# YuanxunLu/LiveSpeechPortraits

Hardware: NVIDIA H100
Metric: 512x512 frames/sec (Feature2Face_G large / May.yaml) (higher is better)
Workload: dtype fp16 hi+lo split operands (3 wgmma MMAs per K step), fp32 accumulate

## Files before the change

livespeechportraits_b200/csrc/conv_wgmma.cuh:

```cuda
#pragma once
#include <cuda_bf16.h>
#include <cuda_fp16.h>
#include "ptx.cuh"

namespace lspg {

constexpr int kTileM = 128;
constexpr int kChunk = 64;
constexpr int kATile = kTileM * 128;
constexpr int kMaxTaps = 9;
constexpr int kThreads = 384;
constexpr int kSmemBudget = 227 * 1024;

struct FastDiv {
  uint32_t mul, shr, d;
};
inline FastDiv make_fast_div(uint32_t d) {
  FastDiv f;
  f.d = d; f.mul = 0; f.shr = 0;
  if (d > 1) {
    uint32_t l = 0;
    while ((1u << l) < d) ++l;
    const uint64_t pw = 31 + l;
    f.mul = static_cast<uint32_t>(((1ull << pw) + d - 1) / d);
    f.shr = static_cast<uint32_t>(pw - 32);
  }
  return f;
}
__device__ __forceinline__ int fast_div(int n, const FastDiv& f) {
  return f.d == 1 ? n : static_cast<int>(__umulhi(static_cast<uint32_t>(n), f.mul) >> f.shr);
}

struct alignas(64) ConvParams {
  const float* scale;
  const float* shift;
  __nv_bfloat16* out_ptr;
  const __nv_bfloat16* res_ptr;
  long long out_limb_stride;
  long long res_limb_stride;
  float* out_f32;
  uint8_t* out_u8;
  float* partial;
  unsigned long long* trace;
  int32_t out_channels, res_channels;
  int32_t out_up;
  int32_t relu, has_res;
  int32_t batch, hs, ws;
  int32_t tw_log2, th_log2;
  int32_t total_tiles;
  int32_t n_split, tiles_per_split;
  int32_t n_tiles;
  int32_t tiles_x, tiles_y, tiles_n;
  int32_t n_phases;
  int32_t trace_skip;
  FastDiv fd_tps, fd_m_tiles, fd_n_tiles, fd_tiles_x, fd_tiles_y;
  int32_t n_taps, n_src;
  int32_t chunks[2];
  int32_t split_len;
  int32_t patch_w, patch_h;
  int32_t desc_base_offset;
  int8_t patch_dx0[4], patch_dy0[4];
  int16_t tap_row[4][kMaxTaps];
  int8_t tap_map[4][kMaxTaps];
  int8_t tap_dx[4][kMaxTaps];
  int8_t tap_dy[4][kMaxTaps];
  CUtensorMap a[4];
  CUtensorMap w;
};

constexpr int kBarBytes = 1024;
constexpr int kTailStride = 17;
template <bool TAIL>
struct AuxCfg {
  static constexpr int kTailBytes = TAIL ? kTileM * kTailStride * 4 : 0;
  static constexpr int kBytes = kBarBytes + kTailBytes;
};

template <int BN, int NL, bool TAIL>
struct ConvCfg {
  using Aux = AuxCfg<TAIL>;
  static constexpr int kBTile = BN * 128;
  static constexpr int kStage = NL * (kATile + kBTile);
  static constexpr int kAvail = kSmemBudget - 1024  - Aux::kBytes;
  static constexpr int kStagesRaw = kAvail / kStage;
  static constexpr int kStages = kStagesRaw > 8 ? 8 : kStagesRaw;
  static constexpr int kSmemBytes = 1024 + kStages * kStage + Aux::kBytes;
  static_assert(kStages >= 2, "pipeline needs at least two stages");
  static_assert(BN == 16 || BN == 64 || BN == 128, "instantiated N tiles");
};

constexpr int kTraceTiles = 12;
constexpr int kTraceSlots = 4 + 8 * kTraceTiles + 4;

struct TileCoord {
  int z, nt, x0, y0, n0, split;
};

__device__ __forceinline__ void trace_stamp(const ConvParams& p, int slot) {
  if (p.trace != nullptr && slot < kTraceSlots) p.trace[static_cast<size_t>(blockIdx.x) * kTraceSlots + slot] = clock64();
}
__device__ __forceinline__ void trace_time(const ConvParams& p, bool at_exit) {
  if (p.trace != nullptr) {
    unsigned long long ns;
    asm volatile("mov.u64 %0, %globaltimer;" : "=l"(ns));
    unsigned long long* t = p.trace + static_cast<size_t>(blockIdx.x) * kTraceSlots;
    t[at_exit ? 3 : 2] = ns;
    if (at_exit) t[4 + 8 * kTraceTiles] = clock64();
  }
}
__device__ __forceinline__ void trace_tile(const ConvParams& p, int lt, int k) {
  if (p.trace != nullptr) {
    const int i = lt - p.trace_skip;
    if (i >= 0 && i < kTraceTiles) p.trace[static_cast<size_t>(blockIdx.x) * kTraceSlots + 4 + 8 * i + k] = clock64();
  }
}

__device__ __forceinline__ TileCoord decode_tile(const ConvParams& p, int t) {
  TileCoord c;
  c.split = fast_div(t, p.fd_tps);
  t -= c.split * p.tiles_per_split;
  const int r = fast_div(t, p.fd_m_tiles);
  const int mt = t - r * static_cast<int>(p.fd_m_tiles.d);
  c.z = fast_div(r, p.fd_n_tiles);
  c.nt = r - c.z * p.n_tiles;
  const int r2 = fast_div(mt, p.fd_tiles_x);
  const int tx = mt - r2 * p.tiles_x;
  const int tn = fast_div(r2, p.fd_tiles_y);
  const int ty = r2 - tn * p.tiles_y;
  c.x0 = tx << p.tw_log2;
  c.y0 = ty << p.th_log2;
  c.n0 = tn << (7 - p.tw_log2 - p.th_log2);
  return c;
}

__device__ __forceinline__ uint32_t pack_bf16x2(float lo, float hi) {
  __nv_bfloat162 v = __floats2bfloat162_rn(lo, hi);
  return *reinterpret_cast<uint32_t*>(&v);
}
__device__ __forceinline__ float bf16_lo(uint32_t u) { return __uint_as_float(u << 16); }
__device__ __forceinline__ float bf16_hi(uint32_t u) { return __uint_as_float(u & 0xFFFF0000u); }

template <bool F16>
__device__ __forceinline__ uint32_t pack2(float lo, float hi) {
  if constexpr (F16) {
    uint32_t r;
    asm("cvt.rn.satfinite.f16x2.f32 %0, %1, %2;" : "=r"(r) : "f"(hi), "f"(lo));
    return r;
  } else {
    return pack_bf16x2(lo, hi);
  }
}
template <bool F16>
__device__ __forceinline__ float unpack_lo(uint32_t u) {
  if constexpr (F16) return __half2float(__ushort_as_half(static_cast<unsigned short>(u & 0xFFFFu)));
  else return bf16_lo(u);
}
template <bool F16>
__device__ __forceinline__ float unpack_hi(uint32_t u) {
  if constexpr (F16) return __half2float(__ushort_as_half(static_cast<unsigned short>(u >> 16)));
  else return bf16_hi(u);
}

__device__ __forceinline__ void row_pixel(const ConvParams& p, const TileCoord& tc, int row, int& n, int& y, int& x) {
  x = tc.x0 + (row & ((1 << p.tw_log2) - 1));
  y = tc.y0 + ((row >> p.tw_log2) & ((1 << p.th_log2) - 1));
  n = tc.n0 + (row >> (p.tw_log2 + p.th_log2));
}

template <int BN, int NL, bool TAIL>
__device__ __forceinline__ void epilogue_regs(const ConvParams& p, const float (&acc)[BN / 2], const TileCoord& tc, int t, int cw,
                                              float* tail_stg) {
  const int wtid = threadIdx.x & 127;
  const int warp = wtid >> 5, lane = wtid & 31;
  const int r0 = cw * 64 + warp * 16 + (lane >> 2);
  const int c0 = 2 * (lane & 3);
  if constexpr (TAIL) {
    float* stg = tail_stg + cw * 64 * kTailStride;
    ptx::named_bar_sync(1 + cw, 128);
#pragma unroll
    for (int j = 0; j < BN / 8; ++j)
#pragma unroll
      for (int h = 0; h < 2; ++h) {
        float* s = stg + (r0 - cw * 64 + 8 * h) * kTailStride + 8 * j + c0;
        s[0] = acc[4 * j + 2 * h];
        s[1] = acc[4 * j + 2 * h + 1];
      }
    ptx::named_bar_sync(1 + cw, 128);
    if (wtid >= 64) return;
    const int row = cw * 64 + wtid;
    const float* v = stg + wtid * kTailStride;
    int pn, py_, px_;
    row_pixel(p, tc, row, pn, py_, px_);
    if (pn >= p.batch || py_ >= p.hs || px_ >= p.ws) return;
    const int oh = 2 * p.hs, ow = 2 * p.ws;
    if (p.out_u8 != nullptr) {
#pragma unroll
      for (int py = 0; py < 2; ++py) {
        uint8_t b[6];
#pragma unroll
        for (int px = 0; px < 2; ++px)
#pragma unroll
          for (int c = 0; c < 3; ++c) {
            const int col = (py * 2 + px) * 3 + c;
            const float vf = tanhf(v[col] * __ldg(p.scale + col) + __ldg(p.shift + col));
            float u = __fmul_rn(__fmul_rn(__fadd_rn(vf, 1.0f), 0.5f), 255.0f);
            u = fminf(fmaxf(u, 0.0f), 255.0f);
            b[px * 3 + c] = static_cast<uint8_t>(static_cast<int>(u));
          }
        uint8_t* dst = p.out_u8 + ((static_cast<size_t>(pn) * oh + (2 * py_ + py)) * ow + 2 * px_) * 3;
        uint16_t* d16 = reinterpret_cast<uint16_t*>(dst);
        d16[0] = static_cast<uint16_t>(b[0] | (b[1] << 8));
        d16[1] = static_cast<uint16_t>(b[2] | (b[3] << 8));
        d16[2] = static_cast<uint16_t>(b[4] | (b[5] << 8));
      }
    } else {
#pragma unroll
      for (int c = 0; c < 3; ++c) {
#pragma unroll
        for (int py = 0; py < 2; ++py) {
          const int c0_ = (py * 2 + 0) * 3 + c, c1_ = (py * 2 + 1) * 3 + c;
          float2 o;
          o.x = tanhf(v[c0_] * __ldg(p.scale + c0_) + __ldg(p.shift + c0_));
          o.y = tanhf(v[c1_] * __ldg(p.scale + c1_) + __ldg(p.shift + c1_));
          float* dst = p.out_f32 + ((static_cast<size_t>(pn) * 3 + c) * oh + (2 * py_ + py)) * ow + 2 * px_;
          *reinterpret_cast<float2*>(dst) = o;
        }
      }
    }
  } else {
    if (p.n_split > 1) {
#pragma unroll
      for (int h = 0; h < 2; ++h) {
        float* dst = p.partial + (static_cast<size_t>(t) * kTileM + r0 + 8 * h) * BN + c0;
#pragma unroll
        for (int j = 0; j < BN / 8; ++j)
          *reinterpret_cast<float2*>(dst + 8 * j) = make_float2(acc[4 * j + 2 * h], acc[4 * j + 2 * h + 1]);
      }
      return;
    }
#pragma unroll
    for (int h = 0; h < 2; ++h) {
      int pn, py_, px_;
      row_pixel(p, tc, r0 + 8 * h, pn, py_, px_);
      if (pn >= p.batch || py_ >= p.hs || px_ >= p.ws) continue;
      const int oh = p.out_up ? 2 * p.hs : p.hs, ow = p.out_up ? 2 * p.ws : p.ws;
      const int oy = p.out_up ? 2 * py_ + (tc.z >> 1) : py_, ox = p.out_up ? 2 * px_ + (tc.z & 1) : px_;
      __nv_bfloat16* out_row = p.out_ptr + ((static_cast<size_t>(pn) * oh + oy) * ow + ox) * p.out_channels + tc.nt * BN + c0;
      const __nv_bfloat16* res_row =
          p.has_res ? p.res_ptr + ((static_cast<size_t>(pn) * p.hs + py_) * p.ws + px_) * p.res_channels + tc.nt * BN + c0 : nullptr;
      const float* sc = p.scale + tc.nt * BN + c0;
      const float* sf = p.shift + tc.nt * BN + c0;
      uint32_t rw[NL][BN / 8];
      if (p.has_res) {
#pragma unroll
        for (int l = 0; l < NL; ++l)
#pragma unroll
          for (int j = 0; j < BN / 8; ++j)
            rw[l][j] = __ldg(reinterpret_cast<const unsigned int*>(res_row + l * p.res_limb_stride + 8 * j));
      }
#pragma unroll
      for (int j = 0; j < BN / 8; ++j) {
        const float2 s2 = __ldg(reinterpret_cast<const float2*>(sc + 8 * j));
        const float2 f2 = __ldg(reinterpret_cast<const float2*>(sf + 8 * j));
        float y0 = fmaf(acc[4 * j + 2 * h], s2.x, f2.x);
        float y1 = fmaf(acc[4 * j + 2 * h + 1], s2.y, f2.y);
        if (p.has_res) {
#pragma unroll
          for (int l = 0; l < NL; ++l) {
            y0 += unpack_lo<NL == 2>(rw[l][j]);
            y1 += unpack_hi<NL == 2>(rw[l][j]);
          }
        }
// ... 68 lines not shown
      }
      __syncwarp();
    }
    ptx::pdl_wait();
    int stage = 0;
    uint32_t phase = 0;
    int issued = 0;
    int lt = 0;
    for (int t = t0; t < p.total_tiles; t += tstep, ++lt) {
      const TileCoord tc = decode_tile(p, t);
      const int kb0 = tc.split * p.split_len;
      const int kb1 = (kb0 + p.split_len < num_kb) ? kb0 + p.split_len : num_kb;
      if (lane == 0) trace_tile(p, lt, 6);
      for (int kb = kb0; kb < kb1; ++kb, ++issued) {
        const int tap = kb / kb_per_tap;
        const int rem = kb - tap * kb_per_tap;
        const int s = (rem < p.chunks[0]) ? 0 : 1;
        const int c = s ? rem - p.chunks[0] : rem;
        const int amap = p.tap_map[tc.z][tap];
        const int xx = tc.x0 + p.tap_dx[tc.z][tap];
        const int yy = tc.y0 + p.tap_dy[tc.z][tap];
        const bool early = issued < pre;
        if (!early) ptx::mbar_wait(&empty_bar[stage], phase ^ 1);
        if (ptx::elect_one()) {
          uint8_t* st = smem + stage * Cfg::kStage;
          if (!early) ptx::mbar_expect_tx(&full_bar[stage], Cfg::kStage);
#pragma unroll
          for (int l = 0; l < NL; ++l) {
            ptx::tma_load_5d(&p.a[amap + s], &full_bar[stage], st + l * kATile, c * kChunk, xx, yy, tc.n0, l);
            if (!early)
              ptx::tma_load_3d(&p.w, &full_bar[stage], st + NL * kATile + l * Cfg::kBTile, kb * kChunk, tc.nt * BN,
                               l * p.n_phases + tc.z);
          }
        }
        __syncwarp();
        if (++stage == Cfg::kStages) { stage = 0; phase ^= 1; }
      }
      if (lane == 0) trace_tile(p, lt, 7);
    }
  } else if (warp >= 4) {
    ptx::pdl_wait();
    const int cw = (warp >> 2) - 1;
    const bool wg_leader = (threadIdx.x & 127) == 0;
    int stage = 0;
    uint32_t phase = 0;
    int lt = 0;
    for (int t = t0; t < p.total_tiles; t += tstep, ++lt) {
      const TileCoord tc = decode_tile(p, t);
      const int kb0 = tc.split * p.split_len;
      const int kb1 = (kb0 + p.split_len < num_kb) ? kb0 + p.split_len : num_kb;
      if (threadIdx.x == 128) trace_tile(p, lt, 0);
      float acc[BN / 2];
#pragma unroll
      for (int i = 0; i < BN / 2; ++i) acc[i] = 0.0f;
      int prev = -1;
      for (int kb = kb0; kb < kb1; ++kb) {
        ptx::mbar_wait(&full_bar[stage], phase);
        if (threadIdx.x == 128 && kb == kb0) trace_tile(p, lt, 1);
        ptx::wgmma_fence();
        const uint32_t a0 = ptx::smem_u32(smem + stage * Cfg::kStage) + cw * 64 * 128;
        const uint32_t b0 = ptx::smem_u32(smem + stage * Cfg::kStage) + NL * kATile;
        const uint64_t a_hi = ptx::gmma_desc_sw128(a0);
        const uint64_t b_hi = ptx::gmma_desc_sw128(b0);
#pragma unroll
        for (int k = 0; k < kChunk / 16; ++k) {
          const uint32_t accum = (kb > kb0 || k > 0) ? 1u : 0u;
          ptx::wgmma_m64k16<BN, NL == 2>(acc, a_hi + 2 * k, b_hi + 2 * k, accum);
          if constexpr (NL == 2) {
            const uint64_t a_lo = ptx::gmma_desc_sw128(a0 + kATile);
            const uint64_t b_lo = ptx::gmma_desc_sw128(b0 + Cfg::kBTile);
            ptx::wgmma_m64k16<BN, true>(acc, a_hi + 2 * k, b_lo + 2 * k, 1u);
            ptx::wgmma_m64k16<BN, true>(acc, a_lo + 2 * k, b_hi + 2 * k, 1u);
          }
        }
        ptx::wgmma_commit();
        ptx::wgmma_wait<1>();
        if (prev >= 0 && wg_leader) release_stage<1>(&empty_bar[prev]);
        prev = stage;
        if (++stage == Cfg::kStages) { stage = 0; phase ^= 1; }
      }
      ptx::wgmma_wait<0>();
      if (prev >= 0 && wg_leader) release_stage<1>(&empty_bar[prev]);
      if (threadIdx.x == 128) trace_tile(p, lt, 2);
      epilogue_regs<BN, NL, TAIL>(p, acc, tc, t, cw, tail_stg);
      if (threadIdx.x == 128) trace_tile(p, lt, 3);
    }
  }
  if (threadIdx.x == 0) trace_time(p, true);
}


constexpr int kPatchSlot = 23 * 1024;
constexpr int kPatchStride = 23 * 1024;

template <int BN, int NL, bool TAIL>
struct PatchCfg {
  using Aux = AuxCfg<TAIL>;
  static constexpr int kBTile = BN * 128;
  static constexpr int kTPS = TAIL ? 9 : (BN >= 128 ? (NL == 1 ? 2 : 1) : (NL == 1 ? 3 : 2));
  static constexpr int kAStage = NL * kPatchStride;
  static constexpr int kBStage = NL * kTPS * kBTile;
  static constexpr int kAStages = 2;
  static constexpr int kAvail = kSmemBudget - 1024 - Aux::kBytes - kAStages * kAStage;
  static constexpr int kBStagesRaw = kAvail / kBStage;
  static constexpr int kBStages = kBStagesRaw > 12 ? 12 : kBStagesRaw;
  static constexpr int kSmemBytes = 1024 + kAStages * kAStage + kBStages * kBStage + Aux::kBytes;
  static_assert(kBStages >= 2, "B ring needs at least two stages");
  static_assert(BN == 16 || BN == 64 || BN == 128, "instantiated N tiles");
};

template <int BN, int NL, bool TAIL, int CL>
__global__ void __launch_bounds__(kThreads, 1) conv_patch_kernel(const __grid_constant__ ConvParams p) {
  using Cfg = PatchCfg<BN, NL, TAIL>;
  const int t0 = static_cast<int>(blockIdx.x), tstep = static_cast<int>(gridDim.x);
  extern __shared__ uint8_t smem_raw[];
  uint8_t* smem = reinterpret_cast<uint8_t*>((reinterpret_cast<uintptr_t>(smem_raw) + 1023) & ~uintptr_t(1023));
  uint8_t* a_ring = smem;
  uint8_t* b_ring = a_ring + Cfg::kAStages * Cfg::kAStage;
  uint8_t* aux = b_ring + Cfg::kBStages * Cfg::kBStage;
  uint64_t* afull_bar = reinterpret_cast<uint64_t*>(aux);
  uint64_t* aempty_bar = afull_bar + Cfg::kAStages;
  uint64_t* bfull_bar = aempty_bar + Cfg::kAStages;
  uint64_t* bempty_bar = bfull_bar + Cfg::kBStages;
  float* tail_stg = reinterpret_cast<float*>(aux + kBarBytes);

  const int warp = __shfl_sync(0xffffffffu, static_cast<int>(threadIdx.x >> 5), 0);
  const int lane = threadIdx.x & 31;
  if (threadIdx.x == 0) { trace_stamp(p, 0); trace_time(p, false); }

  if (warp == 0 && lane == 0) {
    for (int i = 0; i < 4; ++i) ptx::prefetch_tmap(&p.a[i]);
    ptx::prefetch_tmap(&p.w);
    for (int i = 0; i < Cfg::kAStages; ++i) { ptx::mbar_init(&afull_bar[i], 1); ptx::mbar_init(&aempty_bar[i], 2); }
    for (int i = 0; i < Cfg::kBStages; ++i) { ptx::mbar_init(&bfull_bar[i], 1); ptx::mbar_init(&bempty_bar[i], 2 * CL); }
    ptx::fence_mbar_init();
  }
  __syncthreads();
  if (CL > 1) ptx::cluster_sync();
  const uint32_t crank = (CL > 1) ? ptx::cluster_ctarank() : 0u;
  constexpr uint16_t kMask = static_cast<uint16_t>((1u << CL) - 1u);
  ptx::pdl_launch_dependents();
  if (threadIdx.x == 0) trace_stamp(p, 1);

  int kb_per_tap = 0;
  for (int s = 0; s < p.n_src; ++s) kb_per_tap += p.chunks[s];
  const int patch_bytes = p.patch_w * p.patch_h * 128;
  const int n_groups = (p.n_taps + Cfg::kTPS - 1) / Cfg::kTPS;

  if (warp == 0) {
    ptx::pdl_wait();
    int ia = 0, ib = 0;
    uint32_t pha = 0, phb = 0;
    int a_tile = t0, a_ci = -1;
    auto issue_a = [&]() {
      if (a_tile >= p.total_tiles) return;
      const TileCoord tc = decode_tile(p, a_tile);
      const int ci0 = tc.split * p.split_len;
      const int ci1 = (ci0 + p.split_len < kb_per_tap) ? ci0 + p.split_len : kb_per_tap;
      if (a_ci < 0) a_ci = ci0;
      const int s = (a_ci < p.chunks[0]) ? 0 : 1;
      const int c = (s == 0) ? a_ci : a_ci - p.chunks[0];
      ptx::mbar_wait(&aempty_bar[ia], pha ^ 1);
      if (ptx::elect_one()) {
        ptx::mbar_expect_tx(&afull_bar[ia], NL * patch_bytes);
#pragma unroll
        for (int l = 0; l < NL; ++l)
          ptx::tma_load_5d(&p.a[s], &afull_bar[ia], a_ring + ia * Cfg::kAStage + l * kPatchStride, c * kChunk,
                           tc.x0 + p.patch_dx0[tc.z], tc.y0 + p.patch_dy0[tc.z], tc.n0, l);
      }
      __syncwarp();
      if (++ia == Cfg::kAStages) { ia = 0; pha ^= 1; }
      if (++a_ci == ci1) { a_ci = -1; a_tile += tstep; }
    };
    issue_a();
    const int a_after_group = (n_groups > 1) ? 1 : 0;
    int lt = 0;
    for (int t = t0; t < p.total_tiles; t += tstep, ++lt) {
      const TileCoord tc = decode_tile(p, t);
      const int ci0 = tc.split * p.split_len;
      const int ci1 = (ci0 + p.split_len < kb_per_tap) ? ci0 + p.split_len : kb_per_tap;
      if (lane == 0) trace_tile(p, lt, 6);
      for (int ci = ci0; ci < ci1; ++ci) {
        for (int g = 0; g < n_groups; ++g) {
          ptx::mbar_wait(&bempty_bar[ib], phb ^ 1);
          if (ptx::elect_one()) {
            uint8_t* st = b_ring + ib * Cfg::kBStage;
            if constexpr (CL == 1 && NL == 1) {
              ptx::mbar_expect_tx(&bfull_bar[ib], Cfg::kBStage);
              ptx::tma_load_4d(&p.w, &bfull_bar[ib], st, ci * kChunk, tc.nt * BN, g * Cfg::kTPS, tc.z);
            } else {
              const int tap0 = g * Cfg::kTPS;
              const int ntap = (tap0 + Cfg::kTPS < p.n_taps) ? Cfg::kTPS : p.n_taps - tap0;
              ptx::mbar_expect_tx(&bfull_bar[ib], NL * ntap * Cfg::kBTile);
              constexpr int kRows = BN / CL;
              for (int ti = 0; ti < ntap; ++ti)
#pragma unroll
                for (int l = 0; l < NL; ++l) {
                  uint8_t* dst = st + (ti * NL + l) * Cfg::kBTile + crank * kRows * 128;
                  if constexpr (CL == 1)
                    ptx::tma_load_4d(&p.w, &bfull_bar[ib], dst, ci * kChunk, tc.nt * BN, tap0 + ti, l * p.n_phases + tc.z);
                  else
                    ptx::tma_load_4d_mc(&p.w, &bfull_bar[ib], dst, ci * kChunk, tc.nt * BN + crank * kRows, tap0 + ti,
                                        l * p.n_phases + tc.z, kMask);
                }
            }
          }
          __syncwarp();
          if (++ib == Cfg::kBStages) { ib = 0; phb ^= 1; }
          if (g == a_after_group) issue_a();
        }
      }
      if (lane == 0) trace_tile(p, lt, 7);
    }
  } else if (warp >= 4) {
    ptx::pdl_wait();
    const int cw = (warp >> 2) - 1;
    const bool wg_leader = (threadIdx.x & 127) == 0;
    int ia = 0, ib = 0;
    uint32_t pha = 0, phb = 0;
    const uint32_t sbo = static_cast<uint32_t>(p.patch_w) * 128u;
    const uint32_t row_off = static_cast<uint32_t>(cw * 8 * p.patch_w) * 128u;
    const bool boff = p.desc_base_offset != 0;
    int lt = 0;
    for (int t = t0; t < p.total_tiles; t += tstep, ++lt) {
      const TileCoord tc = decode_tile(p, t);
      const int ci0 = tc.split * p.split_len;
      const int ci1 = (ci0 + p.split_len < kb_per_tap) ? ci0 + p.split_len : kb_per_tap;
      if (threadIdx.x == 128) trace_tile(p, lt, 0);
      float acc[BN / 2];
#pragma unroll
      for (int i = 0; i < BN / 2; ++i) acc[i] = 0.0f;
      int prev_b = -1, prev_a = -1;
      for (int ci = ci0; ci < ci1; ++ci) {
        ptx::mbar_wait(&afull_bar[ia], pha);
        const uint32_t a0 = ptx::smem_u32(a_ring + ia * Cfg::kAStage) + row_off;
        for (int g = 0; g < n_groups; ++g) {
          ptx::mbar_wait(&bfull_bar[ib], phb);
          if (threadIdx.x == 128 && ci == ci0 && g == 0) trace_tile(p, lt, 1);
          ptx::wgmma_fence();
          const int tap0 = g * Cfg::kTPS;
          const int tap1 = (tap0 + Cfg::kTPS < p.n_taps) ? tap0 + Cfg::kTPS : p.n_taps;
          const uint32_t b0 = ptx::smem_u32(b_ring + ib * Cfg::kBStage);
          for (int tap = tap0; tap < tap1; ++tap) {
            const uint32_t a_hi_addr = a0 + static_cast<uint32_t>(p.tap_row[tc.z][tap]) * 128u;
            const uint32_t b_hi_addr = b0 + static_cast<uint32_t>(tap - tap0) * (NL * Cfg::kBTile);
            const uint64_t a_hi = ptx::gmma_desc_sw128(a_hi_addr, sbo, boff);
            const uint64_t b_hi = ptx::gmma_desc_sw128(b_hi_addr);
#pragma unroll
            for (int k = 0; k < kChunk / 16; ++k) {
              const uint32_t accum = (ci > ci0 || tap > 0 || k > 0) ? 1u : 0u;
              ptx::wgmma_m64k16<BN, NL == 2>(acc, a_hi + 2 * k, b_hi + 2 * k, accum);
              if constexpr (NL == 2) {
                const uint64_t a_lo = ptx::gmma_desc_sw128(a_hi_addr + kPatchStride, sbo, boff);
                const uint64_t b_lo = ptx::gmma_desc_sw128(b_hi_addr + Cfg::kBTile);
                ptx::wgmma_m64k16<BN, true>(acc, a_hi + 2 * k, b_lo + 2 * k, 1u);
                ptx::wgmma_m64k16<BN, true>(acc, a_lo + 2 * k, b_hi + 2 * k, 1u);
              }
            }
          }
          ptx::wgmma_commit();
          ptx::wgmma_wait<1>();
          if (wg_leader) {
            if (prev_b >= 0) release_stage<CL>(&bempty_bar[prev_b]);
            if (prev_a >= 0) ptx::mbar_arrive(&aempty_bar[prev_a]);
          }
          prev_b = ib;
          prev_a = (g == n_groups - 1) ? ia : -1;
          if (++ib == Cfg::kBStages) { ib = 0; phb ^= 1; }
        }
        if (++ia == Cfg::kAStages) { ia = 0; pha ^= 1; }
      }
      ptx::wgmma_wait<0>();
      if (wg_leader) {
        if (prev_b >= 0) release_stage<CL>(&bempty_bar[prev_b]);
        if (prev_a >= 0) ptx::mbar_arrive(&aempty_bar[prev_a]);
      }
      if (threadIdx.x == 128) trace_tile(p, lt, 2);
      epilogue_regs<BN, NL, TAIL>(p, acc, tc, t, cw, tail_stg);
      if (threadIdx.x == 128) trace_tile(p, lt, 3);
    }
  }
  if (CL > 1) ptx::cluster_sync();
  if (threadIdx.x == 0) trace_time(p, true);
}

struct ReduceParams {
  const float* partial;
  const float* scale;
  const float* shift;
  const __nv_bfloat16* res;
  long long res_limb_stride;
  __nv_bfloat16* out;
  long long out_limb_stride;
  int32_t n_split, tiles_per_split, m_tiles, n_tiles, n_phases;
  int32_t tiles_x, tiles_y, tw_log2, th_log2, bn;
  int32_t batch, hs, ws, up, channels, relu, has_res, nl;
};

__global__ void __launch_bounds__(128) splitk_reduce_kernel(const ReduceParams p) {
  ptx::pdl_wait();
  ptx::pdl_launch_dependents();
  const int groups = p.bn >> 2;
  const long long total = static_cast<long long>(p.tiles_per_split) * kTileM * groups;
  for (long long e = blockIdx.x * static_cast<long long>(blockDim.x) + threadIdx.x; e < total;
       e += static_cast<long long>(gridDim.x) * blockDim.x) {
    const int g = static_cast<int>(e % groups);
    const long long r0 = e / groups;
    const int row = static_cast<int>(r0 % kTileM);
    const int tile = static_cast<int>(r0 / kTileM);
    const int mt = tile % p.m_tiles;
    const int r1 = tile / p.m_tiles;
    const int nt = r1 % p.n_tiles;
    const int z = r1 / p.n_tiles;
    const int tx = mt % p.tiles_x;
    const int r2 = mt / p.tiles_x;
    const int ty = r2 % p.tiles_y;
    const int tn = r2 / p.tiles_y;
    const int tw = row & ((1 << p.tw_log2) - 1);
    const int th = (row >> p.tw_log2) & ((1 << p.th_log2) - 1);
    const int nb = row >> (p.tw_log2 + p.th_log2);
    const int n = (tn << (7 - p.tw_log2 - p.th_log2)) + nb;
    const int y = (ty << p.th_log2) + th, x = (tx << p.tw_log2) + tw;
    if (n >= p.batch || y >= p.hs || x >= p.ws) continue;
    float acc[4] = {0.f, 0.f, 0.f, 0.f};
    const size_t split_stride = static_cast<size_t>(p.tiles_per_split) * kTileM * p.bn;
    const float* src0 = p.partial + (static_cast<size_t>(tile) * kTileM + row) * p.bn + g * 4;
    int s = 0;
    for (; s + 16 <= p.n_split; s += 16) {
      float4 v[16];
#pragma unroll
      for (int u = 0; u < 16; ++u) v[u] = *reinterpret_cast<const float4*>(src0 + (s + u) * split_stride);
#pragma unroll
      for (int u = 0; u < 16; ++u) {
        acc[0] += v[u].x; acc[1] += v[u].y; acc[2] += v[u].z; acc[3] += v[u].w;
      }
    }
    for (; s + 4 <= p.n_split; s += 4) {
      float4 v[4];
#pragma unroll
      for (int u = 0; u < 4; ++u) v[u] = *reinterpret_cast<const float4*>(src0 + (s + u) * split_stride);
#pragma unroll
      for (int u = 0; u < 4; ++u) { acc[0] += v[u].x; acc[1] += v[u].y; acc[2] += v[u].z; acc[3] += v[u].w; }
    }
    for (; s < p.n_split; ++s) {
      const float4 a = *reinterpret_cast<const float4*>(src0 + s * split_stride);
      acc[0] += a.x; acc[1] += a.y; acc[2] += a.z; acc[3] += a.w;
    }
    const int ch = nt * p.bn + g * 4;
    const int oh = p.up ? 2 * p.hs : p.hs, ow = p.up ? 2 * p.ws : p.ws;
    const int oy = p.up ? 2 * y + (z >> 1) : y, ox = p.up ? 2 * x + (z & 1) : x;
    const size_t off = ((static_cast<size_t>(n) * oh + oy) * ow + ox) * p.channels + ch;
    const float4 sc = *reinterpret_cast<const float4*>(p.scale + ch), sh = *reinterpret_cast<const float4*>(p.shift + ch);
    float yv[4] = {fmaf(acc[0], sc.x, sh.x), fmaf(acc[1], sc.y, sh.y), fmaf(acc[2], sc.z, sh.z), fmaf(acc[3], sc.w, sh.w)};
    if (p.has_res) {
      for (int l = 0; l < p.nl; ++l) {
        const uint2 r = *reinterpret_cast<const uint2*>(p.res + l * p.res_limb_stride + off);
        if (p.nl == 2) {
          yv[0] += unpack_lo<true>(r.x); yv[1] += unpack_hi<true>(r.x); yv[2] += unpack_lo<true>(r.y); yv[3] += unpack_hi<true>(r.y);
        } else {
          yv[0] += bf16_lo(r.x); yv[1] += bf16_hi(r.x); yv[2] += bf16_lo(r.y); yv[3] += bf16_hi(r.y);
        }
      }
// ... 22 lines not shown
```

livespeechportraits_b200/csrc/ptx.cuh:

```cuda
#pragma once
#include <cstdint>
#include <cuda.h>

namespace lspg {
namespace ptx {

__device__ __forceinline__ uint32_t smem_u32(const void* p) {
  return static_cast<uint32_t>(__cvta_generic_to_shared(p));
}

__device__ __forceinline__ uint32_t lane_id() {
  uint32_t l;
  asm volatile("mov.u32 %0, %%laneid;" : "=r"(l));
  return l;
}

__device__ __forceinline__ bool elect_one() {
  uint32_t pred = 0;
  asm volatile(
      "{\n\t.reg .b32 rx;\n\t.reg .pred px;\n\t"
      "elect.sync rx|px, %1;\n\t"
      "selp.b32 %0, 1, 0, px;\n\t}"
      : "=r"(pred)
      : "r"(0xFFFFFFFFu));
// ... 44 lines not shown
      if (mbar_try_wait(bar, parity)) return;
    }
    if (globaltimer_ns() - t0 > 4000000000ull) __trap();
  }
}

__device__ __forceinline__ void prefetch_tmap(const CUtensorMap* m) {
  asm volatile("prefetch.tensormap [%0];" ::"l"(reinterpret_cast<uint64_t>(m)) : "memory");
}
__device__ __forceinline__ void tma_load_3d(const CUtensorMap* m, uint64_t* bar, void* dst, int c0, int c1, int c2) {
  asm volatile(
      "cp.async.bulk.tensor.3d.shared::cluster.global.mbarrier::complete_tx::bytes [%0], [%1, {%3, %4, %5}], [%2];"
      ::"r"(smem_u32(dst)), "l"(reinterpret_cast<uint64_t>(m)), "r"(smem_u32(bar)), "r"(c0), "r"(c1), "r"(c2)
      : "memory");
}
__device__ __forceinline__ void tma_load_4d(const CUtensorMap* m, uint64_t* bar, void* dst, int c0, int c1, int c2, int c3) {
  asm volatile(
      "cp.async.bulk.tensor.4d.shared::cluster.global.mbarrier::complete_tx::bytes [%0], [%1, {%3, %4, %5, %6}], [%2];"
      ::"r"(smem_u32(dst)), "l"(reinterpret_cast<uint64_t>(m)), "r"(smem_u32(bar)), "r"(c0), "r"(c1), "r"(c2), "r"(c3)
      : "memory");
}
__device__ __forceinline__ void tma_load_4d_mc(const CUtensorMap* m, uint64_t* bar, void* dst, int c0, int c1, int c2, int c3,
                                               uint16_t mask) {
  asm volatile(
      "cp.async.bulk.tensor.4d.shared::cluster.global.mbarrier::complete_tx::bytes.multicast::cluster"
      " [%0], [%1, {%3, %4, %5, %6}], [%2], %7;"
      ::"r"(smem_u32(dst)), "l"(reinterpret_cast<uint64_t>(m)), "r"(smem_u32(bar)), "r"(c0), "r"(c1), "r"(c2), "r"(c3),
      "h"(mask)
      : "memory");
}
__device__ __forceinline__ void tma_load_5d(const CUtensorMap* m, uint64_t* bar, void* dst, int c0, int c1, int c2,
                                            int c3, int c4) {
  asm volatile(
      "cp.async.bulk.tensor.5d.shared::cluster.global.mbarrier::complete_tx::bytes [%0], [%1, {%3, %4, %5, %6, %7}], [%2];"
      ::"r"(smem_u32(dst)), "l"(reinterpret_cast<uint64_t>(m)), "r"(smem_u32(bar)), "r"(c0), "r"(c1), "r"(c2),
      "r"(c3), "r"(c4)
      : "memory");
}
__device__ __forceinline__ void tma_store_5d(const CUtensorMap* m, const void* src, int c0, int c1, int c2, int c3,
                                             int c4) {
  asm volatile("cp.async.bulk.tensor.5d.global.shared::cta.bulk_group [%0, {%2, %3, %4, %5, %6}], [%1];" ::"l"(
                   reinterpret_cast<uint64_t>(m)),
               "r"(smem_u32(src)), "r"(c0), "r"(c1), "r"(c2), "r"(c3), "r"(c4)
               : "memory");
}
__device__ __forceinline__ void tma_store_commit() { asm volatile("cp.async.bulk.commit_group;" ::: "memory"); }
template <int N>
__device__ __forceinline__ void tma_store_wait_read() {
  asm volatile("cp.async.bulk.wait_group.read %0;" ::"n"(N) : "memory");
}
template <int N>
__device__ __forceinline__ void tma_store_wait_all() {
  asm volatile("cp.async.bulk.wait_group %0;" ::"n"(N) : "memory");
}
__device__ __forceinline__ void fence_proxy_async_smem() { asm volatile("fence.proxy.async.shared::cta;" ::: "memory"); }

__device__ __forceinline__ void cp_async16(void* smem_dst, const void* gmem_src) {
  asm volatile("cp.async.ca.shared.global [%0], [%1], 16;" ::"r"(smem_u32(smem_dst)), "l"(gmem_src) : "memory");
}
__device__ __forceinline__ void cp_async_wait_all() { asm volatile("cp.async.wait_all;" ::: "memory"); }

__device__ __forceinline__ void named_bar_sync(uint32_t id, uint32_t nthreads) {
  asm volatile("bar.sync %0, %1;" ::"r"(id), "r"(nthreads) : "memory");
}

__device__ __forceinline__ void mbar_arrive_cluster(uint64_t* bar, uint32_t cta) {
  asm volatile(
      "{\n\t.reg .b32 ra;\n\t"
      "mapa.shared::cluster.u32 ra, %0, %1;\n\t"
      "mbarrier.arrive.shared::cluster.b64 _, [ra];\n\t}"
      ::"r"(smem_u32(bar)), "r"(cta)
      : "memory");
}

__device__ __forceinline__ uint32_t cluster_ctarank() {
  uint32_t r;
  asm volatile("mov.u32 %0, %%cluster_ctarank;" : "=r"(r));
  return r;
}
__device__ __forceinline__ void cluster_sync() {
  asm volatile("barrier.cluster.arrive.release.aligned;\n\tbarrier.cluster.wait.acquire.aligned;" ::: "memory");
}

__device__ __forceinline__ void wgmma_fence() { asm volatile("wgmma.fence.sync.aligned;" ::: "memory"); }
__device__ __forceinline__ void wgmma_commit() { asm volatile("wgmma.commit_group.sync.aligned;" ::: "memory"); }
template <int N>
__device__ __forceinline__ void wgmma_wait() { asm volatile("wgmma.wait_group.sync.aligned %0;" ::"n"(N) : "memory"); }

__device__ __forceinline__ uint64_t gmma_desc_sw128(uint32_t smem_addr, uint32_t sbo_bytes = 1024, bool base_off = false) {
  uint64_t d = 0;
  d |= static_cast<uint64_t>((smem_addr & 0x3FFFFu) >> 4);
  d |= static_cast<uint64_t>(1) << 16;
  d |= static_cast<uint64_t>(sbo_bytes >> 4) << 32;
  if (base_off) d |= static_cast<uint64_t>((smem_addr >> 7) & 7u) << 49;
  d |= static_cast<uint64_t>(1) << 62;
  return d;
}

__device__ __forceinline__ void wgmma_m64n16_f16(float (&d)[8], uint64_t a_desc, uint64_t b_desc, uint32_t scale_d) {
  asm volatile(
      "{\n\t.reg .pred p;\n\t"
      "setp.ne.b32 p, %10, 0;\n\t"
      "wgmma.mma_async.sync.aligned.m64n16k16.f32.f16.f16 "
      "{%0, %1, %2, %3, %4, %5, %6, %7}, "
      "%8, %9, p, 1, 1, 0, 0;\n\t}"
      : "+f"(d[0]), "+f"(d[1]), "+f"(d[2]), "+f"(d[3]), "+f"(d[4]), "+f"(d[5]), "+f"(d[6]), "+f"(d[7])
      : "l"(a_desc), "l"(b_desc), "r"(scale_d));
}
__device__ __forceinline__ void wgmma_m64n16_bf16(float (&d)[8], uint64_t a_desc, uint64_t b_desc, uint32_t scale_d) {
  asm volatile(
      "{\n\t.reg .pred p;\n\t"
      "setp.ne.b32 p, %10, 0;\n\t"
      "wgmma.mma_async.sync.aligned.m64n16k16.f32.bf16.bf16 "
      "{%0, %1, %2, %3, %4, %5, %6, %7}, "
      "%8, %9, p, 1, 1, 0, 0;\n\t}"
      : "+f"(d[0]), "+f"(d[1]), "+f"(d[2]), "+f"(d[3]), "+f"(d[4]), "+f"(d[5]), "+f"(d[6]), "+f"(d[7])
      : "l"(a_desc), "l"(b_desc), "r"(scale_d));
}
__device__ __forceinline__ void wgmma_m64n64_f16(float (&d)[32], uint64_t a_desc, uint64_t b_desc, uint32_t scale_d) {
  asm volatile(
      "{\n\t.reg .pred p;\n\t"
      "setp.ne.b32 p, %34, 0;\n\t"
      "wgmma.mma_async.sync.aligned.m64n64k16.f32.f16.f16 "
      "{%0, %1, %2, %3, %4, %5, %6, %7, %8, %9, %10, %11, %12, %13, %14, %15, %16, %17, %18, %19, %20, %21, %22, %23, %24, %25, %26, %27, %28, %29, %30, %31}, "
      "%32, %33, p, 1, 1, 0, 0;\n\t}"
      : "+f"(d[0]), "+f"(d[1]), "+f"(d[2]), "+f"(d[3]), "+f"(d[4]), "+f"(d[5]), "+f"(d[6]), "+f"(d[7]), "+f"(d[8]), "+f"(d[9]), "+f"(d[10]), "+f"(d[11]), "+f"(d[12]), "+f"(d[13]), "+f"(d[14]), "+f"(d[15]), "+f"(d[16]), "+f"(d[17]), "+f"(d[18]), "+f"(d[19]), "+f"(d[20]), "+f"(d[21]), "+f"(d[22]), "+f"(d[23]), "+f"(d[24]), "+f"(d[25]), "+f"(d[26]), "+f"(d[27]), "+f"(d[28]), "+f"(d[29]), "+f"(d[30]), "+f"(d[31])
      : "l"(a_desc), "l"(b_desc), "r"(scale_d));
}
__device__ __forceinline__ void wgmma_m64n64_bf16(float (&d)[32], uint64_t a_desc, uint64_t b_desc, uint32_t scale_d) {
  asm volatile(
      "{\n\t.reg .pred p;\n\t"
      "setp.ne.b32 p, %34, 0;\n\t"
      "wgmma.mma_async.sync.aligned.m64n64k16.f32.bf16.bf16 "
      "{%0, %1, %2, %3, %4, %5, %6, %7, %8, %9, %10, %11, %12, %13, %14, %15, %16, %17, %18, %19, %20, %21, %22, %23, %24, %25, %26, %27, %28, %29, %30, %31}, "
      "%32, %33, p, 1, 1, 0, 0;\n\t}"
      : "+f"(d[0]), "+f"(d[1]), "+f"(d[2]), "+f"(d[3]), "+f"(d[4]), "+f"(d[5]), "+f"(d[6]), "+f"(d[7]), "+f"(d[8]), "+f"(d[9]), "+f"(d[10]), "+f"(d[11]), "+f"(d[12]), "+f"(d[13]), "+f"(d[14]), "+f"(d[15]), "+f"(d[16]), "+f"(d[17]), "+f"(d[18]), "+f"(d[19]), "+f"(d[20]), "+f"(d[21]), "+f"(d[22]), "+f"(d[23]), "+f"(d[24]), "+f"(d[25]), "+f"(d[26]), "+f"(d[27]), "+f"(d[28]), "+f"(d[29]), "+f"(d[30]), "+f"(d[31])
      : "l"(a_desc), "l"(b_desc), "r"(scale_d));
}
__device__ __forceinline__ void wgmma_m64n128_f16(float (&d)[64], uint64_t a_desc, uint64_t b_desc, uint32_t scale_d) {
  asm volatile(
      "{\n\t.reg .pred p;\n\t"
      "setp.ne.b32 p, %66, 0;\n\t"
      "wgmma.mma_async.sync.aligned.m64n128k16.f32.f16.f16 "
      "{%0, %1, %2, %3, %4, %5, %6, %7, %8, %9, %10, %11, %12, %13, %14, %15, %16, %17, %18, %19, %20, %21, %22, %23, %24, %25, %26, %27, %28, %29, %30, %31, %32, %33, %34, %35, %36, %37, %38, %39, %40, %41, %42, %43, %44, %45, %46, %47, %48, %49, %50, %51, %52, %53, %54, %55, %56, %57, %58, %59, %60, %61, %62, %63}, "
      "%64, %65, p, 1, 1, 0, 0;\n\t}"
      : "+f"(d[0]), "+f"(d[1]), "+f"(d[2]), "+f"(d[3]), "+f"(d[4]), "+f"(d[5]), "+f"(d[6]), "+f"(d[7]), "+f"(d[8]), "+f"(d[9]), "+f"(d[10]), "+f"(d[11]), "+f"(d[12]), "+f"(d[13]), "+f"(d[14]), "+f"(d[15]), "+f"(d[16]), "+f"(d[17]), "+f"(d[18]), "+f"(d[19]), "+f"(d[20]), "+f"(d[21]), "+f"(d[22]), "+f"(d[23]), "+f"(d[24]), "+f"(d[25]), "+f"(d[26]), "+f"(d[27]), "+f"(d[28]), "+f"(d[29]), "+f"(d[30]), "+f"(d[31]), "+f"(d[32]), "+f"(d[33]), "+f"(d[34]), "+f"(d[35]), "+f"(d[36]), "+f"(d[37]), "+f"(d[38]), "+f"(d[39]), "+f"(d[40]), "+f"(d[41]), "+f"(d[42]), "+f"(d[43]), "+f"(d[44]), "+f"(d[45]), "+f"(d[46]), "+f"(d[47]), "+f"(d[48]), "+f"(d[49]), "+f"(d[50]), "+f"(d[51]), "+f"(d[52]), "+f"(d[53]), "+f"(d[54]), "+f"(d[55]), "+f"(d[56]), "+f"(d[57]), "+f"(d[58]), "+f"(d[59]), "+f"(d[60]), "+f"(d[61]), "+f"(d[62]), "+f"(d[63])
      : "l"(a_desc), "l"(b_desc), "r"(scale_d));
}
__device__ __forceinline__ void wgmma_m64n128_bf16(float (&d)[64], uint64_t a_desc, uint64_t b_desc, uint32_t scale_d) {
  asm volatile(
      "{\n\t.reg .pred p;\n\t"
      "setp.ne.b32 p, %66, 0;\n\t"
      "wgmma.mma_async.sync.aligned.m64n128k16.f32.bf16.bf16 "
      "{%0, %1, %2, %3, %4, %5, %6, %7, %8, %9, %10, %11, %12, %13, %14, %15, %16, %17, %18, %19, %20, %21, %22, %23, %24, %25, %26, %27, %28, %29, %30, %31, %32, %33, %34, %35, %36, %37, %38, %39, %40, %41, %42, %43, %44, %45, %46, %47, %48, %49, %50, %51, %52, %53, %54, %55, %56, %57, %58, %59, %60, %61, %62, %63}, "
      "%64, %65, p, 1, 1, 0, 0;\n\t}"
      : "+f"(d[0]), "+f"(d[1]), "+f"(d[2]), "+f"(d[3]), "+f"(d[4]), "+f"(d[5]), "+f"(d[6]), "+f"(d[7]), "+f"(d[8]), "+f"(d[9]), "+f"(d[10]), "+f"(d[11]), "+f"(d[12]), "+f"(d[13]), "+f"(d[14]), "+f"(d[15]), "+f"(d[16]), "+f"(d[17]), "+f"(d[18]), "+f"(d[19]), "+f"(d[20]), "+f"(d[21]), "+f"(d[22]), "+f"(d[23]), "+f"(d[24]), "+f"(d[25]), "+f"(d[26]), "+f"(d[27]), "+f"(d[28]), "+f"(d[29]), "+f"(d[30]), "+f"(d[31]), "+f"(d[32]), "+f"(d[33]), "+f"(d[34]), "+f"(d[35]), "+f"(d[36]), "+f"(d[37]), "+f"(d[38]), "+f"(d[39]), "+f"(d[40]), "+f"(d[41]), "+f"(d[42]), "+f"(d[43]), "+f"(d[44]), "+f"(d[45]), "+f"(d[46]), "+f"(d[47]), "+f"(d[48]), "+f"(d[49]), "+f"(d[50]), "+f"(d[51]), "+f"(d[52]), "+f"(d[53]), "+f"(d[54]), "+f"(d[55]), "+f"(d[56]), "+f"(d[57]), "+f"(d[58]), "+f"(d[59]), "+f"(d[60]), "+f"(d[61]), "+f"(d[62]), "+f"(d[63])
      : "l"(a_desc), "l"(b_desc), "r"(scale_d));
}

template <int N, bool F16>
__device__ __forceinline__ void wgmma_m64k16(float (&d)[N / 2], uint64_t a_desc, uint64_t b_desc, uint32_t scale_d) {
  static_assert(N == 16 || N == 64 || N == 128, "instantiated N tiles: 16, 64, 128");
  if constexpr (N == 16) { if constexpr (F16) wgmma_m64n16_f16(d, a_desc, b_desc, scale_d); else wgmma_m64n16_bf16(d, a_desc, b_desc, scale_d); }
  if constexpr (N == 64) { if constexpr (F16) wgmma_m64n64_f16(d, a_desc, b_desc, scale_d); else wgmma_m64n64_bf16(d, a_desc, b_desc, scale_d); }
  if constexpr (N == 128) { if constexpr (F16) wgmma_m64n128_f16(d, a_desc, b_desc, scale_d); else wgmma_m64n128_bf16(d, a_desc, b_desc, scale_d); }
}
// ... 4 lines not shown
```

Baseline: 668.7.

## Ping-pong consumer warpgroups over full 128-row tiles in the patch conv kernel

The patch conv kernel's two consumer warpgroups no longer split each tile by rows. Each now owns a whole 128-row tile, holding two 64-row accumulators, and the two alternate tiles. A turn barrier orders their MMA phases so one warpgroup's epilogue can overlap the other's wgmma mainloop. setmaxnreg moves registers from the producer warpgroup to the consumers to hold the doubled accumulator. Tail staging smem is doubled and barrier arrive counts are halved. The costs are higher register pressure, risk of spills at large BN, a larger aux smem footprint that may reduce B-ring stages, and more complex phase bookkeeping.

Result: faster. 709.4 (median of 6 runs) (+6.1%).

```diff
diff --git a/livespeechportraits_b200/csrc/conv_wgmma.cuh b/livespeechportraits_b200/csrc/conv_wgmma.cuh
--- a/livespeechportraits_b200/csrc/conv_wgmma.cuh
+++ b/livespeechportraits_b200/csrc/conv_wgmma.cuh
@@ -70,9 +70,9 @@
 
 constexpr int kBarBytes = 1024;
 constexpr int kTailStride = 17;
-template <bool TAIL>
+template <bool TAIL, int kTailRows = kTileM>
 struct AuxCfg {
-  static constexpr int kTailBytes = TAIL ? kTileM * kTailStride * 4 : 0;
+  static constexpr int kTailBytes = TAIL ? kTailRows * kTailStride * 4 : 0;
   static constexpr int kBytes = kBarBytes + kTailBytes;
 };
 
@@ -168,26 +168,26 @@
 }
 
 template <int BN, int NL, bool TAIL>
-__device__ __forceinline__ void epilogue_regs(const ConvParams& p, const float (&acc)[BN / 2], const TileCoord& tc, int t, int cw,
-                                              float* tail_stg) {
+__device__ __forceinline__ void epilogue_regs(const ConvParams& p, const float (&acc)[BN / 2], const TileCoord& tc, int t, int rb,
+                                              float* tail_stg, int tail_bar) {
   const int wtid = threadIdx.x & 127;
   const int warp = wtid >> 5, lane = wtid & 31;
-  const int r0 = cw * 64 + warp * 16 + (lane >> 2);
+  const int r0 = rb + warp * 16 + (lane >> 2);
   const int c0 = 2 * (lane & 3);
   if constexpr (TAIL) {
-    float* stg = tail_stg + cw * 64 * kTailStride;
-    ptx::named_bar_sync(1 + cw, 128);
+    float* stg = tail_stg;
+    ptx::named_bar_sync(tail_bar, 128);
 #pragma unroll
     for (int j = 0; j < BN / 8; ++j)
 #pragma unroll
       for (int h = 0; h < 2; ++h) {
-        float* s = stg + (r0 - cw * 64 + 8 * h) * kTailStride + 8 * j + c0;
+        float* s = stg + (r0 - rb + 8 * h) * kTailStride + 8 * j + c0;
         s[0] = acc[4 * j + 2 * h];
         s[1] = acc[4 * j + 2 * h + 1];
       }
-    ptx::named_bar_sync(1 + cw, 128);
+    ptx::named_bar_sync(tail_bar, 128);
     if (wtid >= 64) return;
-    const int row = cw * 64 + wtid;
+    const int row = rb + wtid;
     const float* v = stg + wtid * kTailStride;
     int pn, py_, px_;
     row_pixel(p, tc, row, pn, py_, px_);
@@ -422,7 +422,7 @@
       ptx::wgmma_wait<0>();
       if (prev >= 0 && wg_leader) release_stage<1>(&empty_bar[prev]);
       if (threadIdx.x == 128) trace_tile(p, lt, 2);
-      epilogue_regs<BN, NL, TAIL>(p, acc, tc, t, cw, tail_stg);
+      epilogue_regs<BN, NL, TAIL>(p, acc, tc, t, 64 * cw, tail_stg + cw * 64 * kTailStride, 1 + cw);
       if (threadIdx.x == 128) trace_tile(p, lt, 3);
     }
   }
@@ -433,9 +433,13 @@
 constexpr int kPatchSlot = 23 * 1024;
 constexpr int kPatchStride = 23 * 1024;
 
+constexpr int kProducerRegs = 40;
+constexpr int kConsumerRegs = 232;
+static_assert(128 * kProducerRegs + 256 * kConsumerRegs <= 65536, "register file of one SM");
+
 template <int BN, int NL, bool TAIL>
 struct PatchCfg {
-  using Aux = AuxCfg<TAIL>;
+  using Aux = AuxCfg<TAIL, 2 * kTileM>;
   static constexpr int kBTile = BN * 128;
   static constexpr int kTPS = TAIL ? 9 : (BN >= 128 ? (NL == 1 ? 2 : 1) : (NL == 1 ? 3 : 2));
   static constexpr int kAStage = NL * kPatchStride;
@@ -462,6 +466,7 @@
   uint64_t* aempty_bar = afull_bar + Cfg::kAStages;
   uint64_t* bfull_bar = aempty_bar + Cfg::kAStages;
   uint64_t* bempty_bar = bfull_bar + Cfg::kBStages;
+  uint64_t* turn_bar = bempty_bar + Cfg::kBStages;
   float* tail_stg = reinterpret_cast<float*>(aux + kBarBytes);
 
   const int warp = __shfl_sync(0xffffffffu, static_cast<int>(threadIdx.x >> 5), 0);
@@ -471,8 +476,9 @@
   if (warp == 0 && lane == 0) {
     for (int i = 0; i < 4; ++i) ptx::prefetch_tmap(&p.a[i]);
     ptx::prefetch_tmap(&p.w);
-    for (int i = 0; i < Cfg::kAStages; ++i) { ptx::mbar_init(&afull_bar[i], 1); ptx::mbar_init(&aempty_bar[i], 2); }
-    for (int i = 0; i < Cfg::kBStages; ++i) { ptx::mbar_init(&bfull_bar[i], 1); ptx::mbar_init(&bempty_bar[i], 2 * CL); }
+    for (int i = 0; i < Cfg::kAStages; ++i) { ptx::mbar_init(&afull_bar[i], 1); ptx::mbar_init(&aempty_bar[i], 1); }
+    for (int i = 0; i < Cfg::kBStages; ++i) { ptx::mbar_init(&bfull_bar[i], 1); ptx::mbar_init(&bempty_bar[i], CL); }
+    for (int i = 0; i < 2; ++i) ptx::mbar_init(&turn_bar[i], 1);
     ptx::fence_mbar_init();
   }
   __syncthreads();
@@ -487,118 +493,142 @@
   const int patch_bytes = p.patch_w * p.patch_h * 128;
   const int n_groups = (p.n_taps + Cfg::kTPS - 1) / Cfg::kTPS;
 
-  if (warp == 0) {
+  if (warp < 4) {
+    ptx::setmaxnreg_dec<kProducerRegs>();
+    if (warp == 0) {
+      ptx::pdl_wait();
+      int ia = 0, ib = 0;
+      uint32_t pha = 0, phb = 0;
+      int a_tile = t0, a_ci = -1;
+      auto issue_a = [&]() {
+        if (a_tile >= p.total_tiles) return;
+        const TileCoord tc = decode_tile(p, a_tile);
+        const int ci0 = tc.split * p.split_len;
+        const int ci1 = (ci0 + p.split_len < kb_per_tap) ? ci0 + p.split_len : kb_per_tap;
+        if (a_ci < 0) a_ci = ci0;
+        const int s = (a_ci < p.chunks[0]) ? 0 : 1;
+        const int c = (s == 0) ? a_ci : a_ci - p.chunks[0];
+        ptx::mbar_wait(&aempty_bar[ia], pha ^ 1);
+        if (ptx::elect_one()) {
+          ptx::mbar_expect_tx(&afull_bar[ia], NL * patch_bytes);
+#pragma unroll
+          for (int l = 0; l < NL; ++l)
+            ptx::tma_load_5d(&p.a[s], &afull_bar[ia], a_ring + ia * Cfg::kAStage + l * kPatchStride, c * kChunk,
+                             tc.x0 + p.patch_dx0[tc.z], tc.y0 + p.patch_dy0[tc.z], tc.n0, l);
+        }
+        __syncwarp();
+        if (++ia == Cfg::kAStages) { ia = 0; pha ^= 1; }
+        if (++a_ci == ci1) { a_ci = -1; a_tile += tstep; }
+      };
+      issue_a();
+      const int a_after_group = (n_groups > 1) ? 1 : 0;
+      int lt = 0;
+      for (int t = t0; t < p.total_tiles; t += tstep, ++lt) {
+        const TileCoord tc = decode_tile(p, t);
+        const int ci0 = tc.split * p.split_len;
+        const int ci1 = (ci0 + p.split_len < kb_per_tap) ? ci0 + p.split_len : kb_per_tap;
+        if (lane == 0) trace_tile(p, lt, 6);
+        for (int ci = ci0; ci < ci1; ++ci) {
+          for (int g = 0; g < n_groups; ++g) {
+            ptx::mbar_wait(&bempty_bar[ib], phb ^ 1);
+            if (ptx::elect_one()) {
+              uint8_t* st = b_ring + ib * Cfg::kBStage;
+              if constexpr (CL == 1 && NL == 1) {
+                ptx::mbar_expect_tx(&bfull_bar[ib], Cfg::kBStage);
+                ptx::tma_load_4d(&p.w, &bfull_bar[ib], st, ci * kChunk, tc.nt * BN, g * Cfg::kTPS, tc.z);
+              } else {
+                const int tap0 = g * Cfg::kTPS;
+                const int ntap = (tap0 + Cfg::kTPS < p.n_taps) ? Cfg::kTPS : p.n_taps - tap0;
+                ptx::mbar_expect_tx(&bfull_bar[ib], NL * ntap * Cfg::kBTile);
+                constexpr int kRows = BN / CL;
+                for (int ti = 0; ti < ntap; ++ti)
+#pragma unroll
+                  for (int l = 0; l < NL; ++l) {
+                    uint8_t* dst = st + (ti * NL + l) * Cfg::kBTile + crank * kRows * 128;
+                    if constexpr (CL == 1)
+                      ptx::tma_load_4d(&p.w, &bfull_bar[ib], dst, ci * kChunk, tc.nt * BN, tap0 + ti, l * p.n_phases + tc.z);
+                    else
+                      ptx::tma_load_4d_mc(&p.w, &bfull_bar[ib], dst, ci * kChunk, tc.nt * BN + crank * kRows, tap0 + ti,
+                                          l * p.n_phases + tc.z, kMask);
+                  }
+              }
+            }
+            __syncwarp();
+            if (++ib == Cfg::kBStages) { ib = 0; phb ^= 1; }
+            if (g == a_after_group) issue_a();
+          }
+        }
+        if (lane == 0) trace_tile(p, lt, 7);
+      }
+    }
+  } else {
+    ptx::setmaxnreg_inc<kConsumerRegs>();
     ptx::pdl_wait();
+    const int wg = (warp >> 2) - 1;
+    const bool wg_leader = (threadIdx.x & 127) == 0;
     int ia = 0, ib = 0;
     uint32_t pha = 0, phb = 0;
-    int a_tile = t0, a_ci = -1;
-    auto issue_a = [&]() {
-      if (a_tile >= p.total_tiles) return;
-      const TileCoord tc = decode_tile(p, a_tile);
-      const int ci0 = tc.split * p.split_len;
-      const int ci1 = (ci0 + p.split_len < kb_per_tap) ? ci0 + p.split_len : kb_per_tap;
-      if (a_ci < 0) a_ci = ci0;
-      const int s = (a_ci < p.chunks[0]) ? 0 : 1;
-      const int c = (s == 0) ? a_ci : a_ci - p.chunks[0];
-      ptx::mbar_wait(&aempty_bar[ia], pha ^ 1);
-      if (ptx::elect_one()) {
-        ptx::mbar_expect_tx(&afull_bar[ia], NL * patch_bytes);
-#pragma unroll
-        for (int l = 0; l < NL; ++l)
-          ptx::tma_load_5d(&p.a[s], &afull_bar[ia], a_ring + ia * Cfg::kAStage + l * kPatchStride, c * kChunk,
-                           tc.x0 + p.patch_dx0[tc.z], tc.y0 + p.patch_dy0[tc.z], tc.n0, l);
-      }
-      __syncwarp();
-      if (++ia == Cfg::kAStages) { ia = 0; pha ^= 1; }
-      if (++a_ci == ci1) { a_ci = -1; a_tile += tstep; }
-    };
-    issue_a();
-    const int a_after_group = (n_groups > 1) ? 1 : 0;
+    const uint32_t sbo = static_cast<uint32_t>(p.patch_w) * 128u;
+    const uint32_t row_off = static_cast<uint32_t>(8 * p.patch_w) * 128u;
+    const bool boff = p.desc_base_offset != 0;
+    float* stg = tail_stg + wg * kTileM * kTailStride;
     int lt = 0;
     for (int t = t0; t < p.total_tiles; t += tstep, ++lt) {
       const TileCoord tc = decode_tile(p, t);
       const int ci0 = tc.split * p.split_len;
       const int ci1 = (ci0 + p.split_len < kb_per_tap) ? ci0 + p.split_len : kb_per_tap;
-      if (lane == 0) trace_tile(p, lt, 6);
-      for (int ci = ci0; ci < ci1; ++ci) {
-        for (int g = 0; g < n_groups; ++g) {
-          ptx::mbar_wait(&bempty_bar[ib], phb ^ 1);
-          if (ptx::elect_one()) {
-            uint8_t* st = b_ring + ib * Cfg::kBStage;
-            if constexpr (CL == 1 && NL == 1) {
-              ptx::mbar_expect_tx(&bfull_bar[ib], Cfg::kBStage);
-              ptx::tma_load_4d(&p.w, &bfull_bar[ib], st, ci * kChunk, tc.nt * BN, g * Cfg::kTPS, tc.z);
-            } else {
-              const int tap0 = g * Cfg::kTPS;
-              const int ntap = (tap0 + Cfg::kTPS < p.n_taps) ? Cfg::kTPS : p.n_taps - tap0;
-              ptx::mbar_expect_tx(&bfull_bar[ib], NL * ntap * Cfg::kBTile);
-              constexpr int kRows = BN / CL;
-              for (int ti = 0; ti < ntap; ++ti)
-#pragma unroll
-                for (int l = 0; l < NL; ++l) {
-                  uint8_t* dst = st + (ti * NL + l) * Cfg::kBTile + crank * kRows * 128;
-                  if constexpr (CL == 1)
-                    ptx::tma_load_4d(&p.w, &bfull_bar[ib], dst, ci * kChunk, tc.nt * BN, tap0 + ti, l * p.n_phases + tc.z);
-                  else
-                    ptx::tma_load_4d_mc(&p.w, &bfull_bar[ib], dst, ci * kChunk, tc.nt * BN + crank * kRows, tap0 + ti,
-                                        l * p.n_phases + tc.z, kMask);
-                }
-            }
-          }
-          __syncwarp();
-          if (++ib == Cfg::kBStages) { ib = 0; phb ^= 1; }
-          if (g == a_after_group) issue_a();
-        }
-      }
-      if (lane == 0) trace_tile(p, lt, 7);
-    }
-  } else if (warp >= 4) {
-    ptx::pdl_wait();
-    const int cw = (warp >> 2) - 1;
-    const bool wg_leader = (threadIdx.x & 127) == 0;
-    int ia = 0, ib = 0;
-    uint32_t pha = 0, phb = 0;
-    const uint32_t sbo = static_cast<uint32_t>(p.patch_w) * 128u;
-    const uint32_t row_off = static_cast<uint32_t>(cw * 8 * p.patch_w) * 128u;
-    const bool boff = p.desc_base_offset != 0;
-    int lt = 0;
-    for (int t = t0; t < p.total_tiles; t += tstep, ++lt) {
-      const TileCoord tc = decode_tile(p, t);
-      const int ci0 = tc.split * p.split_len;
-      const int ci1 = (ci0 + p.split_len < kb_per_tap) ? ci0 + p.split_len : kb_per_tap;
-      if (threadIdx.x == 128) trace_tile(p, lt, 0);
-      float acc[BN / 2];
-#pragma unroll
-      for (int i = 0; i < BN / 2; ++i) acc[i] = 0.0f;
+      if ((lt & 1) != wg) {
+        ia += ci1 - ci0;
+        pha ^= static_cast<uint32_t>(ia / Cfg::kAStages) & 1u;
+        ia %= Cfg::kAStages;
+        ib += (ci1 - ci0) * n_groups;
+        phb ^= static_cast<uint32_t>(ib / Cfg::kBStages) & 1u;
+        ib %= Cfg::kBStages;
+        continue;
+      }
+      if (lt > 0) ptx::mbar_wait(&turn_bar[wg ^ 1], static_cast<uint32_t>((lt - 1) >> 1) & 1u);
+      if (wg_leader) trace_tile(p, lt, 0);
+      float acc[2][BN / 2];
+#pragma unroll
+      for (int h = 0; h < 2; ++h)
+#pragma unroll
+        for (int i = 0; i < BN / 2; ++i) acc[h][i] = 0.0f;
       int prev_b = -1, prev_a = -1;
       for (int ci = ci0; ci < ci1; ++ci) {
         ptx::mbar_wait(&afull_bar[ia], pha);
-        const uint32_t a0 = ptx::smem_u32(a_ring + ia * Cfg::kAStage) + row_off;
+        const uint32_t a0 = ptx::smem_u32(a_ring + ia * Cfg::kAStage);
         for (int g = 0; g < n_groups; ++g) {
           ptx::mbar_wait(&bfull_bar[ib], phb);
-          if (threadIdx.x == 128 && ci == ci0 && g == 0) trace_tile(p, lt, 1);
+          if (wg_leader && ci == ci0 && g == 0) trace_tile(p, lt, 1);
           ptx::wgmma_fence();
           const int tap0 = g * Cfg::kTPS;
-          const int tap1 = (tap0 + Cfg::kTPS < p.n_taps) ? tap0 + Cfg::kTPS : p.n_taps;
           const uint32_t b0 = ptx::smem_u32(b_ring + ib * Cfg::kBStage);
-          for (int tap = tap0; tap < tap1; ++tap) {
-            const uint32_t a_hi_addr = a0 + static_cast<uint32_t>(p.tap_row[tc.z][tap]) * 128u;
-            const uint32_t b_hi_addr = b0 + static_cast<uint32_t>(tap - tap0) * (NL * Cfg::kBTile);
-            const uint64_t a_hi = ptx::gmma_desc_sw128(a_hi_addr, sbo, boff);
-            const uint64_t b_hi = ptx::gmma_desc_sw128(b_hi_addr);
-#pragma unroll
-            for (int k = 0; k < kChunk / 16; ++k) {
-              const uint32_t accum = (ci > ci0 || tap > 0 || k > 0) ? 1u : 0u;
-              ptx::wgmma_m64k16<BN, NL == 2>(acc, a_hi + 2 * k, b_hi + 2 * k, accum);
-              if constexpr (NL == 2) {
-                const uint64_t a_lo = ptx::gmma_desc_sw128(a_hi_addr + kPatchStride, sbo, boff);
-                const uint64_t b_lo = ptx::gmma_desc_sw128(b_hi_addr + Cfg::kBTile);
-                ptx::wgmma_m64k16<BN, true>(acc, a_hi + 2 * k, b_lo + 2 * k, 1u);
-                ptx::wgmma_m64k16<BN, true>(acc, a_lo + 2 * k, b_hi + 2 * k, 1u);
+#pragma unroll
+          for (int i = 0; i < Cfg::kTPS; ++i) {
+            const int tap = tap0 + i;
+            if (i == 0 || tap < p.n_taps) {
+              const uint32_t a_hi_addr = a0 + static_cast<uint32_t>(p.tap_row[tc.z][tap]) * 128u;
+              const uint32_t b_hi_addr = b0 + static_cast<uint32_t>(i) * (NL * Cfg::kBTile);
+              const uint64_t b_hi = ptx::gmma_desc_sw128(b_hi_addr);
+              const uint64_t b_lo = ptx::gmma_desc_sw128(b_hi_addr + Cfg::kBTile);
+#pragma unroll
+              for (int k = 0; k < kChunk / 16; ++k) {
+                const uint32_t accum = (ci > ci0 || tap > 0 || k > 0) ? 1u : 0u;
+#pragma unroll
+                for (int h = 0; h < 2; ++h) {
+                  const uint64_t a_hi = ptx::gmma_desc_sw128(a_hi_addr + h * row_off, sbo, boff);
+                  ptx::wgmma_m64k16<BN, NL == 2>(acc[h], a_hi + 2 * k, b_hi + 2 * k, accum);
+                  if constexpr (NL == 2) {
+                    const uint64_t a_lo = ptx::gmma_desc_sw128(a_hi_addr + h * row_off + kPatchStride, sbo, boff);
+                    ptx::wgmma_m64k16<BN, true>(acc[h], a_hi + 2 * k, b_lo + 2 * k, 1u);
+                    ptx::wgmma_m64k16<BN, true>(acc[h], a_lo + 2 * k, b_hi + 2 * k, 1u);
+                  }
+                }
               }
             }
           }
           ptx::wgmma_commit();
+          if (ci == ci1 - 1 && g == n_groups - 1 && wg_leader) ptx::mbar_arrive(&turn_bar[wg]);
           ptx::wgmma_wait<1>();
           if (wg_leader) {
             if (prev_b >= 0) release_stage<CL>(&bempty_bar[prev_b]);
@@ -615,9 +645,11 @@
         if (prev_b >= 0) release_stage<CL>(&bempty_bar[prev_b]);
         if (prev_a >= 0) ptx::mbar_arrive(&aempty_bar[prev_a]);
       }
-      if (threadIdx.x == 128) trace_tile(p, lt, 2);
-      epilogue_regs<BN, NL, TAIL>(p, acc, tc, t, cw, tail_stg);
-      if (threadIdx.x == 128) trace_tile(p, lt, 3);
+      if (wg_leader) trace_tile(p, lt, 2);
+#pragma unroll
+      for (int h = 0; h < 2; ++h)
+        epilogue_regs<BN, NL, TAIL>(p, acc[h], tc, t, 64 * h, stg + 64 * h * kTailStride, 1 + wg);
+      if (wg_leader) trace_tile(p, lt, 3);
     }
   }
   if (CL > 1) ptx::cluster_sync();
diff --git a/livespeechportraits_b200/csrc/ptx.cuh b/livespeechportraits_b200/csrc/ptx.cuh
--- a/livespeechportraits_b200/csrc/ptx.cuh
+++ b/livespeechportraits_b200/csrc/ptx.cuh
@@ -150,6 +150,11 @@
   asm volatile("barrier.cluster.arrive.release.aligned;\n\tbarrier.cluster.wait.acquire.aligned;" ::: "memory");
 }
 
+template <uint32_t N>
+__device__ __forceinline__ void setmaxnreg_dec() { asm volatile("setmaxnreg.dec.sync.aligned.u32 %0;" ::"n"(N)); }
+template <uint32_t N>
+__device__ __forceinline__ void setmaxnreg_inc() { asm volatile("setmaxnreg.inc.sync.aligned.u32 %0;" ::"n"(N)); }
+
 __device__ __forceinline__ void wgmma_fence() { asm volatile("wgmma.fence.sync.aligned;" ::: "memory"); }
 __device__ __forceinline__ void wgmma_commit() { asm volatile("wgmma.commit_group.sync.aligned;" ::: "memory"); }
 template <int N>
```
